# tg623623nana/Vehicle_Motion_Planning_with_Obstacles_Avoidance_using_MPC

Hardware: AMD Instinct MI355X
Metric: OBCA MPC steps/sec (batch) at N=5, 3 obs (higher is better)
Workload: dtype f64

## Files before the change

### vehicle_motion_planning_with_obstacles_avoidance_using_mpc_amd/csrc/obca_device.h

```cpp
#ifndef OBCA_DEVICE_H
#define OBCA_DEVICE_H

#include <math.h>
#include <stdint.h>
#include "../../include/obca_mpc.h"

#define OBCA_ACC_MAX0 0.6
#define OBCA_ACC_MAX1 0.5235987755982988
#define OBCA_T_MIN 1e-4

#define OBCA_MU_INIT 0.1
#define OBCA_KAPPA_MU 0.2
#define OBCA_THETA_MU 1.5
#define OBCA_KAPPA_EPS 10.0
#define OBCA_TAU_MIN 0.99
#define OBCA_BOUND_PUSH 1e-2
#define OBCA_BOUND_FRAC 1e-2
#define OBCA_KAPPA_D 1e-5
#define OBCA_KAPPA_SIGMA 1e10
#define OBCA_S_MAX 100.0
#define OBCA_GAMMA_THETA 1e-5
#define OBCA_GAMMA_PHI 1e-8
#define OBCA_DELTA 1.0
#define OBCA_S_THETA 1.1
// ... 72 lines not shown
    t += 4 * obca_even(N1) + 2 * obca_even(2 * np);
    t += 3 * obca_even(2 * np);
    t += obca_even(N1 * M * 2) + obca_even(N1 * M) + obca_even(3 * N1);
    t += obca_even(36 * N1) + obca_even(8 * N1);
    {
        const long long nx = obca_even(n_max), nr = obca_even(R_max), ny = (long long)MW * 4 * np;
        t += obca_even(ny > nx + nr ? ny : nx + nr);
    }
    t += obca_even(36 * N1 > 12 * np ? 36 * N1 : 12 * np) + obca_even(6 * N1) + obca_even(12 * N1) + obca_even(2 * N1) + obca_even(9 * (N1 + 1));
    t += obca_even(32) + obca_even(8);
    const int inst_off = (int)t;
    t += OBCA_INST_DOUBLES;
    return ObcaShapeSizes{n_max, R_max, inst_off, t};
}
#define OBCA_NO_MU_SLOT (1 << 20)
constexpr int obca_r_mu(int N, int nO, int M, int variant) {
    return 3 + 3 * N + (variant == 4 ? 3 : 0) + 2 * (N + 1) + 2 * N + 2 * N + (variant == 4 ? 2 : 0) + (variant == 6 ? 2 : 0) +
           2 * (N + 1) * nO + (N + 1) * M;
}
constexpr int obca_mu_slot(int N, int nO, int M, int nt) {
    int r = obca_r_mu(N, nO, M, 4);
    if (obca_r_mu(N, nO, M, 6) > r) r = obca_r_mu(N, nO, M, 6);
    if (obca_r_mu(N, nO, M, 8) > r) r = obca_r_mu(N, nO, M, 8);
    return (r + nt - 1) / nt;
}
static_assert(obca_mu_slot(5, 3, 6, 64) == 2 && obca_mu_slot(6, 3, 6, 64) == 3 && obca_mu_slot(5, 2, 2, 64) == 2 &&
              obca_mu_slot(5, 5, 14, 64) == 4 && obca_mu_slot(5, 6, 18, 64) == 4, "mu slots of the one-wavefront shapes");
static_assert(obca_mu_slot(20, 3, 6, 256) == 2 && obca_mu_slot(20, 5, 14, 256) == 3, "mu slots of the four-wavefront shapes");
#define OBCA_LDS_CU_BYTES (160 * 1024)
#define OBCA_LDS_STATIC_BYTES 64
constexpr long long obca_soc_doubles(int N, int nO, int M) {
    return obca_even((long long)obca_shape_sizes(N, nO, M).n_max + 2 * (long long)obca_shape_sizes(N, nO, M).R_max + 2 * (long long)(N + 1) * nO);
}
// ... 116 lines not shown
```

### vehicle_motion_planning_with_obstacles_avoidance_using_mpc_amd/csrc/obca_kernel.hip

```cpp

#include <hip/hip_runtime.h>
#include <stdint.h>
#include <math.h>
#include "obca_device.h"

#define SYNC() __syncthreads()

#ifndef OBCA_NT
#define OBCA_NT 64
#endif

#ifdef OBCA_PROFILE
#define PROF_DECL long long prof_last = wall_clock64();
#define PROF(i) { const long long t_ = wall_clock64(); prof_t[i] += t_ - prof_last; prof_last = t_; }
#define RPROF(i) { const long long t_ = wall_clock64(); prof_t[i] += t_ - rlast; rlast = t_; }
__device__ long long* prof_dummy;
#else
#define PROF_DECL
#define PROF(i)
#define RPROF(i)
#endif

namespace {

// ... 121 lines not shown
        const int k = pr / L.nO, i = pr - k * L.nO;
        const int o0 = S.offm[i], o1 = S.offm[i + 1];
        const double* lam = xv + L.il(k);
        const double* A = S.Aobs + (size_t)k * L.M * 2;
        double c0 = 0.0, c1 = 0.0;
        for (int j = o0; j < o1; ++j) {
            c0 += A[2 * j] * lam[j];
            c1 += A[2 * j + 1] * lam[j];
        }
        cc[2 * pr] = c0;
        cc[2 * pr + 1] = c1;
    }
    SYNC();
}

__device__ __forceinline__ double row_value(const Lay& L, const Sh& S, const Inst& in, const double* xv, const double* ct,
                            const double* st, const double* cc, int r) {
    const double T = L.free_T ? xv[L.iT()] : 1.0;
    const double h = T * in.Ts, ih = rcp64(h);
    if (r < L.r_dyn) return xv[r] - in.x0[r];
    if (r < L.r_term) {
        const int q = r - L.r_dyn, k = q / 3, j = q - 3 * k;
        const double* pk = xv + L.ip(k);
        const double* pn = xv + L.ip(k + 1);
        const double* u = xv + L.iu(k);
        const double f = (j == 0) ? u[0] * ct[k] : (j == 1) ? u[0] * st[k] : u[1];
        return pn[j] - pk[j] - h * f;
    }
    if (r < L.r_xb) {
        const int j = r - L.r_term;
        return xv[L.ip(L.N) + j] - S.xref[j * (L.N + 1) + L.N];
    }
    if (r < L.r_ub) {
        const int q = r - L.r_xb;
        return xv[L.ip(q >> 1) + (q & 1)];
    }
    if (r < L.r_acc) {
        const int q = r - L.r_ub;
        return xv[L.iu(q >> 1) + (q & 1)];
    }
    if (r < L.r_T) {
        const int q = r - L.r_acc, k = q >> 1, c = q & 1;
        const double prev = (k == 0) ? in.u0[c] : xv[L.iu(k - 1) + c];
        return (prev - xv[L.iu(k) + c]) * ih;
    }
    if (r < L.r_tx) return T;
    if (r < L.r_norm) return xv[L.ip(L.N) + (r - L.r_tx)];
    if (r < L.r_dist) {
        const int pr = r - L.r_norm;
        return cc[2 * pr] * cc[2 * pr] + cc[2 * pr + 1] * cc[2 * pr + 1];
    }
    if (r < L.r_lam) {
        const int pr = r - L.r_dist, k = pr / L.nO, i = pr - k * L.nO;
        const double* pk = xv + L.ip(k);
        const double tx = pk[0] + ct[k] * in.off, ty = pk[1] + st[k] * in.off;
        const double* mu = xv + L.imu(k) + 4 * i;
        const double* lam = xv + L.il(k);
        const double* b = S.bobs + (size_t)k * L.M;
        double v = -(in.gego[0] * mu[0] + in.gego[1] * mu[1] + in.gego[2] * mu[2] + in.gego[3] * mu[3]) +
                   tx * cc[2 * pr] + ty * cc[2 * pr + 1];
        for (int j = S.offm[i]; j < S.offm[i + 1]; ++j) v -= b[j] * lam[j];
        return v;
    }
    if (r < L.r_mu) {
        const int q = r - L.r_lam, k = q / L.M, j = q - k * L.M;
        return xv[L.il(k) + j];
    }
    {
        const int q = r - L.r_mu, w4 = 4 * L.nO, k = q / w4, j = q - k * w4;
        return xv[L.imu(k) + j];
    }
}

__device__ __forceinline__ void row_bounds(const Lay& L, const Inst& in, int r, double& lo, double& up) {
    const double INF = INFINITY;
    if (r < L.r_xb) { lo = 0.0; up = 0.0; return; }
    if (r < L.r_ub) { const int j = (r - L.r_xb) & 1; lo = in.xL[j]; up = in.xU[j]; return; }
    if (r < L.r_acc) { const int j = (r - L.r_ub) & 1; lo = in.uL[j]; up = in.uU[j]; return; }
    if (r < L.r_T) { const int c = (r - L.r_acc) & 1; const double a = c ? OBCA_ACC_MAX1 : OBCA_ACC_MAX0; lo = -a; up = a; return; }
    if (r < L.r_tx) { if (r == L.r_T) { lo = 0.0; up = INF; } else { lo = OBCA_T_MIN; up = in.Tmax; } return; }
    if (r < L.r_norm) { if (r == L.r_tx) { lo = in.term[0]; up = INF; } else { lo = in.term[1]; up = in.term[2]; } return; }
    if (r < L.r_dist) { lo = -INF; up = 1.0; return; }
    if (r < L.r_lam) { lo = in.dmin; up = INF; return; }
    lo = 0.0; up = INF;
}

__device__ __forceinline__ void rot_value(const Lay& L, const double* xv, const double* ct, const double* st,
                                          const double* cc, int pr, double& e1, double& e2) {
    const int k = pr / L.nO, i = pr - k * L.nO;
    const double* mu = xv + L.imu(k) + 4 * i;
    const double c0 = cc[2 * pr], c1 = cc[2 * pr + 1];
    e1 = mu[0] - mu[2] + ct[k] * c0 + st[k] * c1;
    e2 = mu[1] - mu[3] - st[k] * c0 + ct[k] * c1;
}

template <bool GRAD>
__device__ __forceinline__ double eval_objective(const Lay& L, const Sh& S, const Inst& in, const double* xv, double sf, int lane) {
    const double T = L.free_T ? xv[L.iT()] : 1.0;
// ... 132 lines not shown
            const double* yd = ym + L.r_dyn + 3 * k;
            double u0 = u[0], u1 = u[1], cs = S.ct[k], sn = S.st[k], yd0 = yd[0], yd1 = yd[1], yd2 = yd[2];
            double um0 = xv[L.iu(km)], um1 = xv[L.iu(km) + 1], ya0 = ym[L.r_acc + 2 * k], ya1 = ym[L.r_acc + 2 * k + 1];
            asm volatile("" : "+v"(u0), "+v"(u1), "+v"(cs), "+v"(sn), "+v"(yd0), "+v"(yd1), "+v"(yd2), "+v"(um0), "+v"(um1),
                              "+v"(ya0), "+v"(ya1), "+v"(gT), "+v"(yT0), "+v"(yT1));
            part -= in.Ts * (u0 * cs * yd0 + u0 * sn * yd1 + u1 * yd2);
            part -= ya0 * ((k == 0 ? in.u0[0] : um0) - u0) * iTh;
            part -= ya1 * ((k == 0 ? in.u0[1] : um1) - u1) * iTh;
        }
        part = red_sum(part);
        if (lane == 0) out[L.iT()] = gT + part + (L.N + 1) * (yT0 + yT1);
    }
    SYNC();
}

__device__ __forceinline__ double row_jdx(const Lay& L, const Sh& S, const Inst& in, int r) {
    const double* xv = S.x;
    const double* d = S.dx;
    const double T = L.free_T ? xv[L.iT()] : 1.0;
    const double dT = L.free_T ? d[L.iT()] : 0.0;
    const double h = T * in.Ts, ih = rcp64(h), iTh = ih * rcp64(T);
    if (r < L.r_xb) return d[L.ip(L.N) + (r - L.r_term)];
    if (r < L.r_ub) { const int q = r - L.r_xb; return d[L.ip(q >> 1) + (q & 1)]; }
    if (r < L.r_acc) { const int q = r - L.r_ub; return d[L.iu(q >> 1) + (q & 1)]; }
    if (r < L.r_T) {
        const int q = r - L.r_acc, k = q >> 1, c = q & 1;
        const double prev = (k == 0) ? in.u0[c] : xv[L.iu(k - 1) + c];
        const double dprev = (k == 0) ? 0.0 : d[L.iu(k - 1) + c];
        const double qq = prev - xv[L.iu(k) + c];
        return (dprev - d[L.iu(k) + c]) * ih - qq * iTh * dT;
    }
    if (r < L.r_tx) return dT;
    if (r < L.r_norm) return d[L.ip(L.N) + (r - L.r_tx)];
    if (r < L.r_lam) {
        const bool isn = r < L.r_dist;
        const int pr = isn ? r - L.r_norm : r - L.r_dist;
        const int k = pr / L.nO, i = pr - k * L.nO;
        const double c0 = S.cc[2 * pr], c1 = S.cc[2 * pr + 1];
        const double* A = S.Aobs + (size_t)k * L.M * 2;
        const double* dl = d + L.il(k);
        double s0 = 0.0, s1 = 0.0, sb = 0.0;
        for (int j = S.offm[i]; j < S.offm[i + 1]; ++j) {
            s0 += A[2 * j] * dl[j];
            s1 += A[2 * j + 1] * dl[j];
            sb += S.bobs[(size_t)k * L.M + j] * dl[j];
        }
        if (isn) return 2.0 * (c0 * s0 + c1 * s1);
        const double cs = S.ct[k], sn = S.st[k];
        const double* pk = xv + L.ip(k);
        const double* dp = d + L.ip(k);
        const double* dm = d + L.imu(k) + 4 * i;
        const double tx = pk[0] + cs * in.off, ty = pk[1] + sn * in.off;
        return -(in.gego[0] * dm[0] + in.gego[1] * dm[1] + in.gego[2] * dm[2] + in.gego[3] * dm[3]) + tx * s0 +
               ty * s1 - sb + c0 * dp[0] + c1 * dp[1] + in.off * (-sn * c0 + cs * c1) * dp[2];
    }
    if (r < L.r_mu) { const int q = r - L.r_lam, k = q / L.M; return d[L.il(k) + (q - k * L.M)]; }
    { const int q = r - L.r_mu, w4 = 4 * L.nO, k = q / w4; return d[L.imu(k) + (q - k * w4)]; }
}

#define OBCA_ROW_FIELDS(X) X(s) X(p) X(n) X(zL) X(zU) X(zp) X(zn) X(g) X(dy) X(iDs) X(iDp) X(iDn) X(rs) X(rp) X(rn)
template <int RPL>
struct Rows {
#define X(f) double f##_[RPL];
    OBCA_ROW_FIELDS(X)
#undef X
    __device__ __forceinline__ static constexpr int slots() { return RPL; }
#define X(f) __device__ __forceinline__ double& f(int j) { return f##_[j]; } \
             __device__ __forceinline__ double f(int j) const { return f##_[j]; }
    OBCA_ROW_FIELDS(X)
#undef X
};
// ... 1108 lines not shown
struct ObcaHead {
    int32_t B, N, nO, M, n_max, R_max, inst_off, two_sided, soc_lds;
    const int32_t* variant;
    const double *x0, *u0, *xref, *A, *b, *Ts, *term;
    double *xopt, *uopt, *ts_opt;
    int32_t *status, *iters;
    double *info, *prof, *warm_z;
    const int32_t* warm_use;
    double warm_mu;
    double *cert_z, *cert_y, *soc_ws, *gm_ws;
    long long gm_stride;
};

typedef const __attribute__((address_space(4))) ObcaLaunch ObcaLaunchConst;

struct ShapeAny { static constexpr bool fixed = false; static constexpr int N = 0, nO = 0, M = 0, n_max = 0, R_max = 0, inst_off = 0, soc_lds = 0, mu_slot = OBCA_NO_MU_SLOT; };
template <int N_, int NO_, int M_, bool FT = false>
struct ShapeIs {
    static constexpr bool fixed = true;
    static constexpr int N = N_, nO = NO_, M = M_;
    static constexpr int mu_slot = OBCA_NT == 64 ? obca_mu_slot(N_, NO_, M_, OBCA_NT) : OBCA_NO_MU_SLOT;
    static constexpr int n_max = obca_shape_sizes(N_, NO_, M_).n_max, R_max = obca_shape_sizes(N_, NO_, M_).R_max - (FT ? 3 : 0),
                         inst_off = obca_shape_sizes(N_, NO_, M_).inst_off;
#if OBCA_NT == 64
    static constexpr int RPL = R_max <= 256 ? 4 : R_max <= 320 ? 5 : 6;
    static_assert(R_max <= 384, "shape beyond the one-wavefront kernels");
    static constexpr int soc_lds = obca_soc_lds_wave(N_, NO_, M_);
#else
    static constexpr int RPL = R_max <= 768 ? 3 : -5;
    static_assert(R_max <= 1280, "shape beyond the four-wavefront LDS kernels");
    static constexpr int soc_lds = obca_soc_lds_mw(N_, NO_, M_);
#endif
};

template <int RPL, bool FROM_MEMORY = false, class DESC = const ObcaLaunch, class SHAPE = ShapeAny>
__device__ __forceinline__ void obca_ipm_body(DESC& Ain, const int inst, const bool first) {
    extern __shared__ __attribute__((aligned(16))) double smem[];
    const int lane = threadIdx.x;
    ObcaHead A;
    {
        constexpr bool U = FROM_MEMORY;
        A.B = uni<U>(Ain.B); A.N = uni<U>(Ain.N); A.nO = uni<U>(Ain.nO); A.M = uni<U>(Ain.M); A.n_max = uni<U>(Ain.n_max);
        A.R_max = uni<U>(Ain.R_max); A.inst_off = uni<U>(Ain.inst_off); A.two_sided = uni<U>(Ain.two_sided); A.soc_lds = uni<U>(Ain.soc_lds);
        A.variant = uni<U>(Ain.variant); A.x0 = uni<U>(Ain.x0); A.u0 = uni<U>(Ain.u0); A.xref = uni<U>(Ain.xref); A.A = uni<U>(Ain.A);
        A.b = uni<U>(Ain.b); A.Ts = uni<U>(Ain.Ts); A.term = uni<U>(Ain.term); A.xopt = uni<U>(Ain.xopt); A.uopt = uni<U>(Ain.uopt);
        A.ts_opt = uni<U>(Ain.ts_opt); A.status = uni<U>(Ain.status); A.iters = uni<U>(Ain.iters); A.info = uni<U>(Ain.info);
        A.prof = uni<U>(Ain.prof); A.warm_z = uni<U>(Ain.warm_z); A.warm_use = uni<U>(Ain.warm_use); A.warm_mu = uni<U>(Ain.warm_mu);
        A.cert_z = uni<U>(Ain.cert_z); A.cert_y = uni<U>(Ain.cert_y); A.soc_ws = uni<U>(Ain.soc_ws);
        A.gm_ws = Ain.gm_ws; A.gm_stride = Ain.gm_stride;
        if constexpr (SHAPE::fixed) {
            A.N = SHAPE::N; A.nO = SHAPE::nO; A.M = SHAPE::M; A.n_max = SHAPE::n_max; A.R_max = SHAPE::R_max; A.inst_off = SHAPE::inst_off;
            A.soc_lds = SHAPE::soc_lds;
        }
    }
    if (inst >= A.B) return;
#ifdef OBCA_PROFILE
    const long long prof_body_t0 = wall_clock64();
#endif
    if (A.variant[inst] == 0) {
        if (lane == 0) { A.status[inst] = OBCA_STATUS_SKIPPED; A.iters[inst] = 0; }
        return;
    }
    {
        const int v = A.variant[inst];
        if ((v != 4 && v != 6 && v != 8) || (v == 6 && A.term == nullptr)) {
            if (lane == 0 && first) { A.status[inst] = OBCA_STATUS_BAD_VARIANT; A.iters[inst] = 0; }
            return;
        }
    }
    __shared__ int ladder_state[4];
    __shared__ double ladder_f;
    const int order = OBCA_EFFECTIVE_ORDER(Ain.prm.opt.order, A.variant[inst], A.warm_z != nullptr && (A.warm_use == nullptr || A.warm_use[inst] != 0), Ain.prm.opt.nstarts == 1);
    int start_s = 0, escalated = 0, held_bits = 0;
    if (!first) {
        const int st0 = __builtin_amdgcn_readfirstlane(A.status[inst]);
        if (st0 == OBCA_STATUS_OK || st0 == OBCA_STATUS_ACCEPTABLE || st0 < OBCA_STATUS_NUMERIC) return;
        const int l0 = __builtin_amdgcn_readfirstlane(ladder_state[0]);
        escalated = l0 & 15; held_bits = l0 & 0xf20;
        start_s = __builtin_amdgcn_readfirstlane(ladder_state[3]);
        if (A.variant[inst] == 4 && (l0 & 16) && escalated < OBCA_N_ESCALATIONS) ++escalated;
        else { escalated = 0; if (++start_s >= Ain.prm.opt.nstarts + ((Ain.prm.opt.dodge && A.variant[inst] != 4) ? OBCA_DODGE_PASSES(A.variant[inst]) : 0)) return; }
    }
    const double rho_mult = escalated ? OBCA_RHO_ESCALATION(escalated) : 1.0;
    const int kind = start_s < Ain.prm.opt.nstarts ? OBCA_START_KIND(order, start_s) : (((start_s - Ain.prm.opt.nstarts) & 1) == 0 ? OBCA_KIND_DODGE_R : OBCA_KIND_DODGE_L);
    const bool dodge2 = start_s >= Ain.prm.opt.nstarts + 2;
    const bool from_window = kind == OBCA_KIND_WINDOW;

    Lay L;
    L.N = A.N; L.nO = A.nO; L.M = A.M;
    L.variant = A.variant[inst];
    L.free_T = (L.variant == 4) ? 1 : 0;
    L.NS = 5 + L.M + 4 * L.nO;
    L.n = (L.N + 1) * (3 + L.M + 4 * L.nO) + 2 * L.N + L.free_T;
    L.npair = (L.N + 1) * L.nO;
    L.r_init = 0; L.r_dyn = 3; L.r_term = 3 + 3 * L.N;
    L.r_xb = L.r_term + (L.variant == 4 ? 3 : 0);
    L.r_ub = L.r_xb + 2 * (L.N + 1);
    L.r_acc = L.r_ub + 2 * L.N;
    L.r_T = L.r_acc + 2 * L.N;
    L.r_tx = L.r_T + (L.free_T ? 2 : 0);
    L.r_norm = L.r_tx + (L.variant == 6 ? 2 : 0);
    L.r_dist = L.r_norm + L.npair;
    L.r_lam = L.r_dist + L.npair;
    L.r_mu = L.r_lam + (L.N + 1) * L.M;
    L.R = L.r_mu + (L.N + 1) * 4 * L.nO;

    constexpr bool GM = (RPL == 0);
    constexpr int MUS = SHAPE::mu_slot;
    Sh S;
    Rows<RPL> W;
    {
        double* p = smem;
        double* q = nullptr;
        if constexpr (GM) q = A.gm_ws + (size_t)blockIdx.x * (size_t)A.gm_stride;
        auto take = [&](int cnt) { double* r = p; p += (cnt + 1) & ~1; return r; };
        auto takeG = [&](int cnt) { if constexpr (!GM) { double* r = p; p += (cnt + 1) & ~1; return r; } else { double* r = q; q += (cnt + 1) & ~1; return r; } };
        const int nmax = A.n_max, Rmax = A.R_max, np = L.npair, N1 = L.N + 1;
        S.x = takeG(nmax); S.dx = takeG(nmax > 120 ? nmax : 120); S.gf = take(5 * N1 + 1); S.bx = takeG(nmax);
        S.y = takeG(Rmax); S.Einv = takeG(Rmax); S.gh = takeG(Rmax); S.Lb = takeG(Rmax); S.Ub = takeG(Rmax); S.dy = take(3 * N1 + 3);
        S.ct = take(N1); S.st = take(N1); S.cc = takeG(2 * np); S.ctt = take(N1); S.stt = take(N1); S.cct = takeG(2 * np);
// ... 125 lines not shown
    eval_geom(L, S, S.x, S.ct, S.st, S.cc, lane);
    double f0 = eval_objective<true>(L, S, in, S.x, 1.0, lane);
    {
        double gm = 0.0;
        for (int t = lane; t <= L.igT(); t += NT) gm = dmaxabs(gm, S.gf[t]);
        gm = fmax(red_max(gm), O.rho);
        sf = (gm > OBCA_MAX_GRADIENT) ? OBCA_MAX_GRADIENT / gm : 1.0;
        rho = O.rho * sf;
    }
    SYNC();
    f0 = eval_objective<true>(L, S, in, S.x, sf, lane);
    PUT(IV_F, f0);
    double mu = (from_window || (kind >= OBCA_KIND_DODGE_R && !dodge2)) ? OBCA_RESTART_MU : (warm ? A.warm_mu : (dodge2 ? OBCA_DODGE_LEVEL2_MU : OBCA_MU_INIT));
    {
        int bb = 0;
        for (int r = lane; r < L.R; r += NT) {
            double lo, up;
            row_bounds(L, in, r, lo, up);
            S.Lb[r] = lo; S.Ub[r] = up;
            S.tmp[r] = row_value(L, S, in, S.x, S.ct, S.st, S.cc, r);
        }
#pragma unroll
        for (int j = 0; j < W.slots(); ++j) {
            const int r = lane + NT * j;
            W.s(j) = 0.0; W.p(j) = 1.0; W.n(j) = 1.0;
            W.zL(j) = 0.0; W.zU(j) = 0.0; W.zp(j) = 1.0; W.zn(j) = 1.0; W.g(j) = 0.0; W.dy(j) = 0.0;
            W.iDs(j) = 0.0; W.iDp(j) = 1.0; W.iDn(j) = 1.0; W.rs(j) = 0.0; W.rp(j) = 0.0; W.rn(j) = 0.0;
            if (r < L.R) {
                const bool muk = mu_only<MUS>(j);
                const double lo = muk ? 0.0 : S.Lb[r], up = muk ? INFINITY : S.Ub[r];
// ... 199 lines not shown
            if (!bad || soc_pass) break;
            if (first_try) {
                delta_w = (dw_last == 0.0) ? OBCA_DELTA_W_0 : fmax(OBCA_DELTA_W_MIN, OBCA_KAPPA_W_MINUS * dw_last);
                first_try = false;
            } else {
                delta_w *= (dw_last == 0.0) ? OBCA_KAPPA_W_PLUS_BAR : OBCA_KAPPA_W_PLUS;
            }
            if (delta_w > OBCA_DELTA_W_MAX) { fail = 1; break; }
        }
        if (fail) { status = OBCA_STATUS_NUMERIC; break; }
        if (!soc_pass && delta_w > 0.0) PUT(IV_DWLAST, delta_w);
        double a_max = 1.0, a_z = 1.0, dphi = 0.0, phi = 0.0;
        const double phik = GET(IV_PHIK);
        const bool phi_known = !soc_pass && isfinite(phik);
        const double tau = GET(IV_TAU);
        for (int r = lane; r < L.R; r += NT)
            S.tmp[r] = row_soft(L, r) ? S.dy[r] : (row_jdx(L, S, in, r) + S.gh[r]) * S.Einv[r];
#if OBCA_NT == 64
        PROF(19)
#endif
#pragma unroll
        for (int j = 0; j < W.slots(); ++j) {
            const int r = lane + NT * j;
            if (r < L.R) {
                const bool muk = mu_only<MUS>(j);
                const bool eq = muk ? false : row_iseq(L, r);
                const double lo_ = muk ? 0.0 : S.Lb[r], up_ = muk ? INFINITY : S.Ub[r];
                const bool hasL = !eq && lo_ > -INFINITY, hasU = !eq && up_ < INFINITY;
                const double dy = S.tmp[r];
                W.dy(j) = dy;
// ... 58 lines not shown
        } else {
            a_try = a_max;
            a_z = S.lsv[LS_AZ]; dphi = S.lsv[LS_DPHI]; phi = S.lsv[LS_PHI]; alpha_min = S.lsv[LS_AMIN];
            pw_th = S.lsv[LS_PWTH]; pw_dphi = S.lsv[LS_PWDPHI]; alpha = S.lsv[LS_ALPHA]; th_old = S.lsv[LS_THOLD];
        }
        soc_pass = false;
        PROF(6)
        double f_t = 0.0, phi_acc = NAN;
        bool accepted = false, aug = false;
        for (;;) {
            for (int t = lane; t < L.n; t += NT) S.xt[t] = S.x[t] + a_try * S.dx[t];
            SYNC();
            eval_geom(L, S, S.xt, S.ctt, S.stt, S.cct, lane);
            f_t = eval_objective<true>(L, S, in, S.xt, sf, lane);
            double th_t = 0.0, phi_t = 0.0;
            for (int r = lane; r < L.R; r += NT) S.tmp[r] = row_value(L, S, in, S.xt, S.ctt, S.stt, S.cct, r);
#pragma unroll
            for (int j = 0; j < W.slots(); ++j) {
                const int r = lane + NT * j;
                if (r < L.R) {
                    const bool muk = mu_only<MUS>(j);
                    const bool eq = muk ? false : row_iseq(L, r);
                    const double dy = W.dy(j), w = muk ? 1.0 : row_w(L, r);
                    const double lo_ = muk ? 0.0 : S.Lb[r], up_ = muk ? INFINITY : S.Ub[r];
                    const double st = eq ? 0.0 : W.s(j) + a_try * (dy - W.rs(j)) * W.iDs(j);
                    const double pt = W.p(j) + a_try * (dy - W.rp(j)) * W.iDp(j);
                    const double nt = W.n(j) + a_try * (-dy - W.rn(j)) * W.iDn(j);
                    const double gt = S.tmp[r];
                    th_t += w * fabs(gt - st - pt + nt);
                    phi_t += w * row_barrier(lo_, up_, eq, st, pt, nt, mu, rho);
// ... 260 lines not shown
        const int NSs = 5 + a->M + 4 * a->nO, nn = N1 * (3 + a->M + 4 * a->nO) + 2 * a->N;
        for (int t = lane; t < nn; t += nt) { const int k = t / NSs, q = t - k * NSs; zc[t] = q < 3 ? x0s[q] : 0.0; }
    }
    if (a->cert_y != nullptr) {
        double* yc = a->cert_y + (size_t)inst * (a->R_max + 2 * N1 * a->nO);
        const int Rv = 3 + 3 * a->N + 2 * N1 + 4 * a->N + 2 + N1 * (2 * a->nO + a->M + 4 * a->nO);
        for (int t = lane; t < Rv + 2 * N1 * a->nO; t += nt) yc[t] = 0.0;
    }
    if (lane == 0) {
        a->ts_opt[inst] = ts; a->status[inst] = OBCA_STATUS_INFEASIBLE; a->iters[inst] = 0;
        if (a->info) { double* io = a->info + (size_t)inst * 4; io[0] = 0.0; io[1] = sh; io[2] = 0.0; io[3] = 0.0; }
    }
    return 1;
}

template <int RPL, bool LOOP, class DESC, class SHAPE = ShapeAny>
__device__ __forceinline__ void solve_passes(DESC& A, DESC& A2, DESC& A3) {
    const int inst = blockIdx.x;
    __shared__ int drv_scr;
    {
        extern __shared__ __attribute__((aligned(16))) double smem[];
        const int scr = terminal_screen_dev((const ObcaLaunch*)__builtin_amdgcn_kernarg_segment_ptr(), inst, threadIdx.x, blockDim.x,
                                            &reinterpret_cast<Inst*>(smem + A.inst_off)->Tmax);
        if (scr == 1) return;
        if (threadIdx.x == 0) drv_scr = scr;
    }
    if constexpr (LOOP) {
        if (inst >= A.B) return;
#pragma clang loop unroll(disable)
        for (int pass = 0; pass < OBCA_MAX_PASSES; ++pass) {
            obca_ipm_body<RPL, false, DESC, SHAPE>(A, inst, pass == 0);
            __syncthreads();
            const int st = A.status[inst];
            if (st == OBCA_STATUS_OK || st == OBCA_STATUS_ACCEPTABLE || st < OBCA_STATUS_NUMERIC) return;
            if (drv_scr == 2 && pass + 1 == A.prm.opt.nstarts) return;
        }
    } else {
        static_assert(OBCA_MAX_PASSES == 9, "one inlined copy of the body per pass");
        obca_ipm_body<RPL, false, DESC, SHAPE>(A, inst, true);
        if (inst >= A.B) return;
        __syncthreads();
        {
            const int st = A2.status[inst];
            if (st == OBCA_STATUS_OK || st == OBCA_STATUS_ACCEPTABLE || st < OBCA_STATUS_NUMERIC) return;
        }
        if (drv_scr == 2 && A2.prm.opt.nstarts == 1) return;
        obca_ipm_body<RPL, false, DESC, SHAPE>(A2, inst, false);
        __syncthreads();
        obca_ipm_body<RPL, false, DESC, SHAPE>(A3, inst, false);
        __syncthreads();
// ... 33 lines not shown
#ifndef OBCA_LOOP_GM
#define OBCA_LOOP_GM true
#endif
#if OBCA_NT == 64 && defined(OBCA_TU_SHAPE)
#ifndef OBCA_SHAPE_KERNEL_ATTR
#define OBCA_SHAPE_KERNEL_ATTR
#endif
#define OBCA_DEFINE_SHAPE_KERNEL(N_, O_, M_)                                                                                   \
    extern "C" __global__ void __launch_bounds__(64) OBCA_SHAPE_KERNEL_ATTR obca_ipm_kernel_s##N_##_##O_##_##M_(ObcaLaunch A, ObcaLaunch A2, ObcaLaunch A3) { \
        using SH = ShapeIs<N_, O_, M_>;                                                                                        \
        solve_with_escalation<SH::RPL, true, true, SH>(A, A2, A3);                                                            \
    }
OBCA_TU_SHAPE(OBCA_DEFINE_SHAPE_KERNEL)
#elif OBCA_NT == 64
extern "C" int obca_internal_mu_slot(int N, int nO, int M, int nt) { return obca_mu_slot(N, nO, M, nt); }
extern "C" __global__ void __launch_bounds__(64) obca_ipm_kernel_r4(ObcaLaunch A, ObcaLaunch A2, ObcaLaunch A3) { solve_with_escalation<4, OBCA_LOOP_R4>(A, A2, A3); }
extern "C" __global__ void __launch_bounds__(64) obca_ipm_kernel_r5(ObcaLaunch A, ObcaLaunch A2, ObcaLaunch A3) { solve_with_escalation<5, OBCA_LOOP_R56>(A, A2, A3); }
extern "C" __global__ void __launch_bounds__(64) obca_ipm_kernel_r6(ObcaLaunch A, ObcaLaunch A2, ObcaLaunch A3) { solve_with_escalation<6, OBCA_LOOP_R56>(A, A2, A3); }
extern "C" __global__ void __launch_bounds__(64) obca_ipm_kernel_gm1(ObcaLaunch A, ObcaLaunch A2, ObcaLaunch A3) { solve_with_escalation<0, OBCA_LOOP_GM>(A, A2, A3); }

#include "obca_rollout_core.h"
#include "obca_audit_core.h"

__device__ __noinline__ void ro_prepare(const rollout::Dev* D, int b) { rollout::prepare(*D, b); }
__device__ __noinline__ void ro_finish(const rollout::Dev* D, int b) { rollout::finish(*D, b); }
__device__ __noinline__ void ro_stop(const rollout::Dev* D, int b) { rollout::stop_check_wave(*D, b); }
__device__ __noinline__ int ro_screen(const ObcaLaunch* L, int b, double* tmax) { return terminal_screen_dev(L, b, 0, 1, tmax); }
__device__ __noinline__ int ro_retry(const rollout::Dev* D, int g, int b) { rollout::make_retry(*D, g, b); return D->var8[g][b]; }
__device__ __noinline__ long long ro_flag_sel(const rollout::Dev* D, int b) { return ((long long)D->sel[b] << 32) | (unsigned)D->flags[b]; }

// ... 173 lines not shown
```

Baseline: 1.206 million.

## Specialize IPM body per variant with compile-time row-kind dispatch

Adds per-variant template instantiations of the fixed-shape IPM body, so the row layout becomes compile-time constant. Row evaluation loops are split into a mixed prefix and a pure-mu tail, each with a compile-time mask of the row kinds it can hold. This lets the compiler drop impossible branches in row_value, row_bounds and row_jdx. It is meant to remove per-row branch chains and runtime layout arithmetic, at the cost of three inlined body copies, which adds code size and may raise register pressure.

```diff
diff --git a/vehicle_motion_planning_with_obstacles_avoidance_using_mpc_amd/csrc/obca_device.h b/vehicle_motion_planning_with_obstacles_avoidance_using_mpc_amd/csrc/obca_device.h
--- a/vehicle_motion_planning_with_obstacles_avoidance_using_mpc_amd/csrc/obca_device.h
+++ b/vehicle_motion_planning_with_obstacles_avoidance_using_mpc_amd/csrc/obca_device.h
@@ -110,9 +110,44 @@
     return ObcaShapeSizes{n_max, R_max, inst_off, t};
 }
 #define OBCA_NO_MU_SLOT (1 << 20)
-constexpr int obca_r_mu(int N, int nO, int M, int variant) {
-    return 3 + 3 * N + (variant == 4 ? 3 : 0) + 2 * (N + 1) + 2 * N + 2 * N + (variant == 4 ? 2 : 0) + (variant == 6 ? 2 : 0) +
-           2 * (N + 1) * nO + (N + 1) * M;
+struct ObcaRowLayout { int r_init, r_dyn, r_term, r_xb, r_ub, r_acc, r_T, r_tx, r_norm, r_dist, r_lam, r_mu, R, n, free_T; };
+constexpr ObcaRowLayout obca_row_layout(int N, int nO, int M, int variant) {
+    ObcaRowLayout l{};
+    l.free_T = variant == 4 ? 1 : 0;
+    l.n = (N + 1) * (3 + M + 4 * nO) + 2 * N + l.free_T;
+    l.r_init = 0; l.r_dyn = 3; l.r_term = 3 + 3 * N;
+    l.r_xb = l.r_term + (variant == 4 ? 3 : 0);
+    l.r_ub = l.r_xb + 2 * (N + 1);
+    l.r_acc = l.r_ub + 2 * N;
+    l.r_T = l.r_acc + 2 * N;
+    l.r_tx = l.r_T + (variant == 4 ? 2 : 0);
+    l.r_norm = l.r_tx + (variant == 6 ? 2 : 0);
+    l.r_dist = l.r_norm + (N + 1) * nO;
+    l.r_lam = l.r_dist + (N + 1) * nO;
+    l.r_mu = l.r_lam + (N + 1) * M;
+    l.R = l.r_mu + (N + 1) * 4 * nO;
+    return l;
+}
+constexpr int obca_r_mu(int N, int nO, int M, int variant) { return obca_row_layout(N, nO, M, variant).r_mu; }
+enum { OBCA_KIND_BIT_INIT = 1, OBCA_KIND_BIT_DYN = 2, OBCA_KIND_BIT_TERM = 4, OBCA_KIND_BIT_XB = 8, OBCA_KIND_BIT_UB = 16, OBCA_KIND_BIT_ACC = 32,
+       OBCA_KIND_BIT_T = 64, OBCA_KIND_BIT_TX = 128, OBCA_KIND_BIT_NORM = 256, OBCA_KIND_BIT_DIST = 512, OBCA_KIND_BIT_LAM = 1024,
+       OBCA_KIND_BIT_MU = 2048, OBCA_KIND_BITS_ALL = 4095 };
+constexpr int obca_slot_kinds(int N, int nO, int M, int variant, int nt, int j) {
+    const ObcaRowLayout l = obca_row_layout(N, nO, M, variant);
+    const int first[13] = {l.r_init, l.r_dyn, l.r_term, l.r_xb, l.r_ub, l.r_acc, l.r_T, l.r_tx, l.r_norm, l.r_dist, l.r_lam, l.r_mu, l.R};
+    const int lo = nt * j, hi = nt * j + nt < l.R ? nt * j + nt : l.R;
+    int kinds = 0;
+    for (int k = 0; k < 12; ++k) {
+        const int a = first[k] > lo ? first[k] : lo, b = first[k + 1] < hi ? first[k + 1] : hi;
+        if (a < b) kinds |= 1 << k;
+    }
+    return kinds;
+}
+constexpr int obca_own_mu_slot(int N, int nO, int M, int variant, int nt) { return (obca_r_mu(N, nO, M, variant) + nt - 1) / nt; }
+constexpr int obca_mixed_kinds(int N, int nO, int M, int variant, int nt) {
+    int kinds = 0;
+    for (int j = 0; j < obca_own_mu_slot(N, nO, M, variant, nt); ++j) kinds |= obca_slot_kinds(N, nO, M, variant, nt, j);
+    return kinds;
 }
 constexpr int obca_mu_slot(int N, int nO, int M, int nt) {
     int r = obca_r_mu(N, nO, M, 4);
diff --git a/vehicle_motion_planning_with_obstacles_avoidance_using_mpc_amd/csrc/obca_kernel.hip b/vehicle_motion_planning_with_obstacles_avoidance_using_mpc_amd/csrc/obca_kernel.hip
--- a/vehicle_motion_planning_with_obstacles_avoidance_using_mpc_amd/csrc/obca_kernel.hip
+++ b/vehicle_motion_planning_with_obstacles_avoidance_using_mpc_amd/csrc/obca_kernel.hip
@@ -2,6 +2,7 @@
 #include <hip/hip_runtime.h>
 #include <stdint.h>
 #include <math.h>
+#include <type_traits>
 #include "obca_device.h"
 
 #define SYNC() __syncthreads()
@@ -159,12 +160,18 @@
     SYNC();
 }
 
+#define OBCA_ROW_IS(K, bound) ((KM & (K)) != 0 && ((KM & ~(2 * (K) - 1)) == 0 || r < (bound)))
+template <int KM = OBCA_KIND_BITS_ALL>
 __device__ __forceinline__ double row_value(const Lay& L, const Sh& S, const Inst& in, const double* xv, const double* ct,
                             const double* st, const double* cc, int r) {
+    if constexpr (KM == OBCA_KIND_BIT_MU) {
+        const int q = r - L.r_mu, w4 = 4 * L.nO, k = q / w4, j = q - k * w4;
+        return xv[L.imu(k) + j];
+    }
     const double T = L.free_T ? xv[L.iT()] : 1.0;
     const double h = T * in.Ts, ih = rcp64(h);
-    if (r < L.r_dyn) return xv[r] - in.x0[r];
-    if (r < L.r_term) {
+    if (OBCA_ROW_IS(OBCA_KIND_BIT_INIT, L.r_dyn)) return xv[r] - in.x0[r];
+    if (OBCA_ROW_IS(OBCA_KIND_BIT_DYN, L.r_term)) {
         const int q = r - L.r_dyn, k = q / 3, j = q - 3 * k;
         const double* pk = xv + L.ip(k);
         const double* pn = xv + L.ip(k + 1);
@@ -172,30 +179,30 @@
         const double f = (j == 0) ? u[0] * ct[k] : (j == 1) ? u[0] * st[k] : u[1];
         return pn[j] - pk[j] - h * f;
     }
-    if (r < L.r_xb) {
+    if (OBCA_ROW_IS(OBCA_KIND_BIT_TERM, L.r_xb)) {
         const int j = r - L.r_term;
         return xv[L.ip(L.N) + j] - S.xref[j * (L.N + 1) + L.N];
     }
-    if (r < L.r_ub) {
+    if (OBCA_ROW_IS(OBCA_KIND_BIT_XB, L.r_ub)) {
         const int q = r - L.r_xb;
         return xv[L.ip(q >> 1) + (q & 1)];
     }
-    if (r < L.r_acc) {
+    if (OBCA_ROW_IS(OBCA_KIND_BIT_UB, L.r_acc)) {
         const int q = r - L.r_ub;
         return xv[L.iu(q >> 1) + (q & 1)];
     }
-    if (r < L.r_T) {
+    if (OBCA_ROW_IS(OBCA_KIND_BIT_ACC, L.r_T)) {
         const int q = r - L.r_acc, k = q >> 1, c = q & 1;
         const double prev = (k == 0) ? in.u0[c] : xv[L.iu(k - 1) + c];
         return (prev - xv[L.iu(k) + c]) * ih;
     }
-    if (r < L.r_tx) return T;
-    if (r < L.r_norm) return xv[L.ip(L.N) + (r - L.r_tx)];
-    if (r < L.r_dist) {
+    if (OBCA_ROW_IS(OBCA_KIND_BIT_T, L.r_tx)) return T;
+    if (OBCA_ROW_IS(OBCA_KIND_BIT_TX, L.r_norm)) return xv[L.ip(L.N) + (r - L.r_tx)];
+    if (OBCA_ROW_IS(OBCA_KIND_BIT_NORM, L.r_dist)) {
         const int pr = r - L.r_norm;
         return cc[2 * pr] * cc[2 * pr] + cc[2 * pr + 1] * cc[2 * pr + 1];
     }
-    if (r < L.r_lam) {
+    if (OBCA_ROW_IS(OBCA_KIND_BIT_DIST, L.r_lam)) {
         const int pr = r - L.r_dist, k = pr / L.nO, i = pr - k * L.nO;
         const double* pk = xv + L.ip(k);
         const double tx = pk[0] + ct[k] * in.off, ty = pk[1] + st[k] * in.off;
@@ -207,7 +214,7 @@
         for (int j = S.offm[i]; j < S.offm[i + 1]; ++j) v -= b[j] * lam[j];
         return v;
     }
-    if (r < L.r_mu) {
+    if (OBCA_ROW_IS(OBCA_KIND_BIT_LAM, L.r_mu)) {
         const int q = r - L.r_lam, k = q / L.M, j = q - k * L.M;
         return xv[L.il(k) + j];
     }
@@ -217,16 +224,18 @@
     }
 }
 
+template <int KM = OBCA_KIND_BITS_ALL>
 __device__ __forceinline__ void row_bounds(const Lay& L, const Inst& in, int r, double& lo, double& up) {
     const double INF = INFINITY;
-    if (r < L.r_xb) { lo = 0.0; up = 0.0; return; }
-    if (r < L.r_ub) { const int j = (r - L.r_xb) & 1; lo = in.xL[j]; up = in.xU[j]; return; }
-    if (r < L.r_acc) { const int j = (r - L.r_ub) & 1; lo = in.uL[j]; up = in.uU[j]; return; }
-    if (r < L.r_T) { const int c = (r - L.r_acc) & 1; const double a = c ? OBCA_ACC_MAX1 : OBCA_ACC_MAX0; lo = -a; up = a; return; }
-    if (r < L.r_tx) { if (r == L.r_T) { lo = 0.0; up = INF; } else { lo = OBCA_T_MIN; up = in.Tmax; } return; }
-    if (r < L.r_norm) { if (r == L.r_tx) { lo = in.term[0]; up = INF; } else { lo = in.term[1]; up = in.term[2]; } return; }
-    if (r < L.r_dist) { lo = -INF; up = 1.0; return; }
-    if (r < L.r_lam) { lo = in.dmin; up = INF; return; }
+    constexpr int EQ = OBCA_KIND_BIT_INIT | OBCA_KIND_BIT_DYN | OBCA_KIND_BIT_TERM;
+    if ((KM & EQ) != 0 && ((KM & ~EQ) == 0 || r < L.r_xb)) { lo = 0.0; up = 0.0; return; }
+    if (OBCA_ROW_IS(OBCA_KIND_BIT_XB, L.r_ub)) { const int j = (r - L.r_xb) & 1; lo = in.xL[j]; up = in.xU[j]; return; }
+    if (OBCA_ROW_IS(OBCA_KIND_BIT_UB, L.r_acc)) { const int j = (r - L.r_ub) & 1; lo = in.uL[j]; up = in.uU[j]; return; }
+    if (OBCA_ROW_IS(OBCA_KIND_BIT_ACC, L.r_T)) { const int c = (r - L.r_acc) & 1; const double a = c ? OBCA_ACC_MAX1 : OBCA_ACC_MAX0; lo = -a; up = a; return; }
+    if (OBCA_ROW_IS(OBCA_KIND_BIT_T, L.r_tx)) { if (r == L.r_T) { lo = 0.0; up = INF; } else { lo = OBCA_T_MIN; up = in.Tmax; } return; }
+    if (OBCA_ROW_IS(OBCA_KIND_BIT_TX, L.r_norm)) { if (r == L.r_tx) { lo = in.term[0]; up = INF; } else { lo = in.term[1]; up = in.term[2]; } return; }
+    if (OBCA_ROW_IS(OBCA_KIND_BIT_NORM, L.r_dist)) { lo = -INF; up = 1.0; return; }
+    if (OBCA_ROW_IS(OBCA_KIND_BIT_DIST, L.r_lam)) { lo = in.dmin; up = INF; return; }
     lo = 0.0; up = INF;
 }
 
@@ -389,26 +398,28 @@
     SYNC();
 }
 
+template <int KM = OBCA_KIND_BITS_ALL>
 __device__ __forceinline__ double row_jdx(const Lay& L, const Sh& S, const Inst& in, int r) {
     const double* xv = S.x;
     const double* d = S.dx;
+    if constexpr (KM == OBCA_KIND_BIT_MU) { const int q = r - L.r_mu, w4 = 4 * L.nO, k = q / w4; return d[L.imu(k) + (q - k * w4)]; }
     const double T = L.free_T ? xv[L.iT()] : 1.0;
     const double dT = L.free_T ? d[L.iT()] : 0.0;
     const double h = T * in.Ts, ih = rcp64(h), iTh = ih * rcp64(T);
-    if (r < L.r_xb) return d[L.ip(L.N) + (r - L.r_term)];
-    if (r < L.r_ub) { const int q = r - L.r_xb; return d[L.ip(q >> 1) + (q & 1)]; }
-    if (r < L.r_acc) { const int q = r - L.r_ub; return d[L.iu(q >> 1) + (q & 1)]; }
-    if (r < L.r_T) {
+    if (OBCA_ROW_IS(OBCA_KIND_BIT_TERM, L.r_xb)) return d[L.ip(L.N) + (r - L.r_term)];
+    if (OBCA_ROW_IS(OBCA_KIND_BIT_XB, L.r_ub)) { const int q = r - L.r_xb; return d[L.ip(q >> 1) + (q & 1)]; }
+    if (OBCA_ROW_IS(OBCA_KIND_BIT_UB, L.r_acc)) { const int q = r - L.r_ub; return d[L.iu(q >> 1) + (q & 1)]; }
+    if (OBCA_ROW_IS(OBCA_KIND_BIT_ACC, L.r_T)) {
         const int q = r - L.r_acc, k = q >> 1, c = q & 1;
         const double prev = (k == 0) ? in.u0[c] : xv[L.iu(k - 1) + c];
         const double dprev = (k == 0) ? 0.0 : d[L.iu(k - 1) + c];
         const double qq = prev - xv[L.iu(k) + c];
         return (dprev - d[L.iu(k) + c]) * ih - qq * iTh * dT;
     }
-    if (r < L.r_tx) return dT;
-    if (r < L.r_norm) return d[L.ip(L.N) + (r - L.r_tx)];
-    if (r < L.r_lam) {
-        const bool isn = r < L.r_dist;
+    if (OBCA_ROW_IS(OBCA_KIND_BIT_T, L.r_tx)) return dT;
+    if (OBCA_ROW_IS(OBCA_KIND_BIT_TX, L.r_norm)) return d[L.ip(L.N) + (r - L.r_tx)];
+    if ((KM & (OBCA_KIND_BIT_NORM | OBCA_KIND_BIT_DIST)) != 0 && ((KM & (OBCA_KIND_BIT_LAM | OBCA_KIND_BIT_MU)) == 0 || r < L.r_lam)) {
+        const bool isn = (KM & OBCA_KIND_BIT_NORM) != 0 && ((KM & OBCA_KIND_BIT_DIST) == 0 || r < L.r_dist);
         const int pr = isn ? r - L.r_norm : r - L.r_dist;
         const int k = pr / L.nO, i = pr - k * L.nO;
         const double c0 = S.cc[2 * pr], c1 = S.cc[2 * pr + 1];
@@ -429,7 +440,7 @@
         return -(in.gego[0] * dm[0] + in.gego[1] * dm[1] + in.gego[2] * dm[2] + in.gego[3] * dm[3]) + tx * s0 +
                ty * s1 - sb + c0 * dp[0] + c1 * dp[1] + in.off * (-sn * c0 + cs * c1) * dp[2];
     }
-    if (r < L.r_mu) { const int q = r - L.r_lam, k = q / L.M; return d[L.il(k) + (q - k * L.M)]; }
+    if (OBCA_ROW_IS(OBCA_KIND_BIT_LAM, L.r_mu)) { const int q = r - L.r_lam, k = q / L.M; return d[L.il(k) + (q - k * L.M)]; }
     { const int q = r - L.r_mu, w4 = 4 * L.nO, k = q / w4; return d[L.imu(k) + (q - k * w4)]; }
 }
 
@@ -1568,11 +1579,17 @@
 
 typedef const __attribute__((address_space(4))) ObcaLaunch ObcaLaunchConst;
 
-struct ShapeAny { static constexpr bool fixed = false; static constexpr int N = 0, nO = 0, M = 0, n_max = 0, R_max = 0, inst_off = 0, soc_lds = 0, mu_slot = OBCA_NO_MU_SLOT; };
-template <int N_, int NO_, int M_, bool FT = false>
+struct ShapeAny {
+    static constexpr bool fixed = false, per_variant = false;
+    static constexpr int N = 0, nO = 0, M = 0, n_max = 0, R_max = 0, inst_off = 0, soc_lds = 0, mu_slot = OBCA_NO_MU_SLOT, variant = 0;
+};
+template <int N_, int NO_, int M_, bool FT = false, int V_ = 0>
 struct ShapeIs {
+    static_assert(V_ == 0 || V_ == 4 || V_ == 6 || V_ == 8, "variant: 4, 6, 8 or 0 (run time)");
     static constexpr bool fixed = true;
-    static constexpr int N = N_, nO = NO_, M = M_;
+    static constexpr int N = N_, nO = NO_, M = M_, variant = V_;
+    static constexpr bool per_variant = OBCA_NT == 64 && !FT && V_ == 0;
+    template <int V> using with_variant = ShapeIs<N_, NO_, M_, FT, V>;
     static constexpr int mu_slot = OBCA_NT == 64 ? obca_mu_slot(N_, NO_, M_, OBCA_NT) : OBCA_NO_MU_SLOT;
     static constexpr int n_max = obca_shape_sizes(N_, NO_, M_).n_max, R_max = obca_shape_sizes(N_, NO_, M_).R_max - (FT ? 3 : 0),
                          inst_off = obca_shape_sizes(N_, NO_, M_).inst_off;
@@ -1586,6 +1603,17 @@
     static constexpr int soc_lds = obca_soc_lds_mw(N_, NO_, M_);
 #endif
 };
+
+template <class SHAPE, class F>
+__device__ __forceinline__ void mixed_then_mu(int lane, F f) {
+    constexpr ObcaRowLayout K = obca_row_layout(SHAPE::N, SHAPE::nO, SHAPE::M, SHAPE::variant);
+    constexpr int MUSV = obca_own_mu_slot(SHAPE::N, SHAPE::nO, SHAPE::M, SHAPE::variant, NT), MIXED = NT * MUSV < K.R ? NT * MUSV : K.R;
+    constexpr int MIX = obca_mixed_kinds(SHAPE::N, SHAPE::nO, SHAPE::M, SHAPE::variant, NT);
+#pragma unroll 1
+    for (int r = lane; r < MIXED; r += NT) f(std::integral_constant<int, MIX>{}, r);
+#pragma unroll 1
+    for (int r = lane + NT * MUSV; r < K.R; r += NT) f(std::integral_constant<int, OBCA_KIND_BIT_MU>{}, r);
+}
 
 template <int RPL, bool FROM_MEMORY = false, class DESC = const ObcaLaunch, class SHAPE = ShapeAny>
 __device__ __forceinline__ void obca_ipm_body(DESC& Ain, const int inst, const bool first) {
@@ -1611,20 +1639,23 @@
 #ifdef OBCA_PROFILE
     const long long prof_body_t0 = wall_clock64();
 #endif
-    if (A.variant[inst] == 0) {
-        if (lane == 0) { A.status[inst] = OBCA_STATUS_SKIPPED; A.iters[inst] = 0; }
-        return;
-    }
-    {
-        const int v = A.variant[inst];
-        if ((v != 4 && v != 6 && v != 8) || (v == 6 && A.term == nullptr)) {
-            if (lane == 0 && first) { A.status[inst] = OBCA_STATUS_BAD_VARIANT; A.iters[inst] = 0; }
+    auto variant_of = [&]() __attribute__((always_inline)) -> int { if constexpr (SHAPE::variant != 0) return SHAPE::variant; else return A.variant[inst]; };
+    if constexpr (SHAPE::variant == 0) {
+        if (A.variant[inst] == 0) {
+            if (lane == 0) { A.status[inst] = OBCA_STATUS_SKIPPED; A.iters[inst] = 0; }
             return;
+        }
+        {
+            const int v = A.variant[inst];
+            if ((v != 4 && v != 6 && v != 8) || (v == 6 && A.term == nullptr)) {
+                if (lane == 0 && first) { A.status[inst] = OBCA_STATUS_BAD_VARIANT; A.iters[inst] = 0; }
+                return;
+            }
         }
     }
     __shared__ int ladder_state[4];
     __shared__ double ladder_f;
-    const int order = OBCA_EFFECTIVE_ORDER(Ain.prm.opt.order, A.variant[inst], A.warm_z != nullptr && (A.warm_use == nullptr || A.warm_use[inst] != 0), Ain.prm.opt.nstarts == 1);
+    const int order = OBCA_EFFECTIVE_ORDER(Ain.prm.opt.order, variant_of(), A.warm_z != nullptr && (A.warm_use == nullptr || A.warm_use[inst] != 0), Ain.prm.opt.nstarts == 1);
     int start_s = 0, escalated = 0, held_bits = 0;
     if (!first) {
         const int st0 = __builtin_amdgcn_readfirstlane(A.status[inst]);
@@ -1632,8 +1663,8 @@
         const int l0 = __builtin_amdgcn_readfirstlane(ladder_state[0]);
         escalated = l0 & 15; held_bits = l0 & 0xf20;
         start_s = __builtin_amdgcn_readfirstlane(ladder_state[3]);
-        if (A.variant[inst] == 4 && (l0 & 16) && escalated < OBCA_N_ESCALATIONS) ++escalated;
-        else { escalated = 0; if (++start_s >= Ain.prm.opt.nstarts + ((Ain.prm.opt.dodge && A.variant[inst] != 4) ? OBCA_DODGE_PASSES(A.variant[inst]) : 0)) return; }
+        if (variant_of() == 4 && (l0 & 16) && escalated < OBCA_N_ESCALATIONS) ++escalated;
+        else { escalated = 0; if (++start_s >= Ain.prm.opt.nstarts + ((Ain.prm.opt.dodge && variant_of() != 4) ? OBCA_DODGE_PASSES(variant_of()) : 0)) return; }
     }
     const double rho_mult = escalated ? OBCA_RHO_ESCALATION(escalated) : 1.0;
     const int kind = start_s < Ain.prm.opt.nstarts ? OBCA_START_KIND(order, start_s) : (((start_s - Ain.prm.opt.nstarts) & 1) == 0 ? OBCA_KIND_DODGE_R : OBCA_KIND_DODGE_L);
@@ -1642,7 +1673,7 @@
 
     Lay L;
     L.N = A.N; L.nO = A.nO; L.M = A.M;
-    L.variant = A.variant[inst];
+    L.variant = variant_of();
     L.free_T = (L.variant == 4) ? 1 : 0;
     L.NS = 5 + L.M + 4 * L.nO;
     L.n = (L.N + 1) * (3 + L.M + 4 * L.nO) + 2 * L.N + L.free_T;
@@ -1658,6 +1689,12 @@
     L.r_lam = L.r_dist + L.npair;
     L.r_mu = L.r_lam + (L.N + 1) * L.M;
     L.R = L.r_mu + (L.N + 1) * 4 * L.nO;
+    if constexpr (SHAPE::variant != 0) {
+        constexpr ObcaRowLayout K = obca_row_layout(SHAPE::N, SHAPE::nO, SHAPE::M, SHAPE::variant);
+        L.free_T = K.free_T; L.n = K.n;
+        L.r_init = K.r_init; L.r_dyn = K.r_dyn; L.r_term = K.r_term; L.r_xb = K.r_xb; L.r_ub = K.r_ub; L.r_acc = K.r_acc; L.r_T = K.r_T;
+        L.r_tx = K.r_tx; L.r_norm = K.r_norm; L.r_dist = K.r_dist; L.r_lam = K.r_lam; L.r_mu = K.r_mu; L.R = K.R;
+    }
 
     constexpr bool GM = (RPL == 0);
     constexpr int MUS = SHAPE::mu_slot;
@@ -1813,6 +1850,15 @@
     double mu = (from_window || (kind >= OBCA_KIND_DODGE_R && !dodge2)) ? OBCA_RESTART_MU : (warm ? A.warm_mu : (dodge2 ? OBCA_DODGE_LEVEL2_MU : OBCA_MU_INIT));
     {
         int bb = 0;
+        if constexpr (SHAPE::variant != 0) {
+            mixed_then_mu<SHAPE>(lane, [&](auto km, int r) __attribute__((always_inline)) {
+                constexpr int KM = decltype(km)::value;
+                double lo, up;
+                row_bounds<KM>(L, in, r, lo, up);
+                S.Lb[r] = lo; S.Ub[r] = up;
+                S.tmp[r] = row_value<KM>(L, S, in, S.x, S.ct, S.st, S.cc, r);
+            });
+        } else
         for (int r = lane; r < L.R; r += NT) {
             double lo, up;
             row_bounds(L, in, r, lo, up);
@@ -2042,6 +2088,13 @@
         const double phik = GET(IV_PHIK);
         const bool phi_known = !soc_pass && isfinite(phik);
         const double tau = GET(IV_TAU);
+        if constexpr (SHAPE::variant != 0) {
+            mixed_then_mu<SHAPE>(lane, [&](auto km, int r) __attribute__((always_inline)) {
+                constexpr int KM = decltype(km)::value, SOFT = OBCA_KIND_BIT_INIT | OBCA_KIND_BIT_DYN;
+                const bool soft = (KM & SOFT) != 0 && ((KM & ~SOFT) == 0 || row_soft(L, r));
+                S.tmp[r] = soft ? S.dy[r] : (row_jdx<KM>(L, S, in, r) + S.gh[r]) * S.Einv[r];
+            });
+        } else
         for (int r = lane; r < L.R; r += NT)
             S.tmp[r] = row_soft(L, r) ? S.dy[r] : (row_jdx(L, S, in, r) + S.gh[r]) * S.Einv[r];
 #if OBCA_NT == 64
@@ -2130,6 +2183,11 @@
             eval_geom(L, S, S.xt, S.ctt, S.stt, S.cct, lane);
             f_t = eval_objective<true>(L, S, in, S.xt, sf, lane);
             double th_t = 0.0, phi_t = 0.0;
+            if constexpr (SHAPE::variant != 0) {
+                mixed_then_mu<SHAPE>(lane, [&](auto km, int r) __attribute__((always_inline)) {
+                    S.tmp[r] = row_value<decltype(km)::value>(L, S, in, S.xt, S.ctt, S.stt, S.cct, r);
+                });
+            } else
             for (int r = lane; r < L.R; r += NT) S.tmp[r] = row_value(L, S, in, S.xt, S.ctt, S.stt, S.cct, r);
 #pragma unroll
             for (int j = 0; j < W.slots(); ++j) {
@@ -2420,6 +2478,17 @@
     return 1;
 }
 
+template <int RPL, class DESC, class SHAPE>
+__device__ __forceinline__ void pass_loop(DESC& A, const int inst, const int* drv_scr) {
+#pragma clang loop unroll(disable)
+    for (int pass = 0; pass < OBCA_MAX_PASSES; ++pass) {
+        obca_ipm_body<RPL, false, DESC, SHAPE>(A, inst, pass == 0);
+        __syncthreads();
+        const int st = A.status[inst];
+        if (st == OBCA_STATUS_OK || st == OBCA_STATUS_ACCEPTABLE || st < OBCA_STATUS_NUMERIC) return;
+        if (*drv_scr == 2 && pass + 1 == A.prm.opt.nstarts) return;
+    }
+}
 template <int RPL, bool LOOP, class DESC, class SHAPE = ShapeAny>
 __device__ __forceinline__ void solve_passes(DESC& A, DESC& A2, DESC& A3) {
     const int inst = blockIdx.x;
@@ -2433,13 +2502,24 @@
     }
     if constexpr (LOOP) {
         if (inst >= A.B) return;
+        if constexpr (SHAPE::per_variant) {
+            const int v = A.variant[inst];
+            if (v == 0 || (v != 4 && v != 6 && v != 8) || (v == 6 && A.term == nullptr)) {
+                if (threadIdx.x == 0) { A.status[inst] = v == 0 ? OBCA_STATUS_SKIPPED : OBCA_STATUS_BAD_VARIANT; A.iters[inst] = 0; }
+                return;
+            }
+            if (v == 4) pass_loop<RPL, DESC, typename SHAPE::template with_variant<4>>(A, inst, &drv_scr);
+            else if (v == 6) pass_loop<RPL, DESC, typename SHAPE::template with_variant<6>>(A, inst, &drv_scr);
+            else pass_loop<RPL, DESC, typename SHAPE::template with_variant<8>>(A, inst, &drv_scr);
+        } else {
 #pragma clang loop unroll(disable)
-        for (int pass = 0; pass < OBCA_MAX_PASSES; ++pass) {
-            obca_ipm_body<RPL, false, DESC, SHAPE>(A, inst, pass == 0);
-            __syncthreads();
-            const int st = A.status[inst];
-            if (st == OBCA_STATUS_OK || st == OBCA_STATUS_ACCEPTABLE || st < OBCA_STATUS_NUMERIC) return;
-            if (drv_scr == 2 && pass + 1 == A.prm.opt.nstarts) return;
+            for (int pass = 0; pass < OBCA_MAX_PASSES; ++pass) {
+                obca_ipm_body<RPL, false, DESC, SHAPE>(A, inst, pass == 0);
+                __syncthreads();
+                const int st = A.status[inst];
+                if (st == OBCA_STATUS_OK || st == OBCA_STATUS_ACCEPTABLE || st < OBCA_STATUS_NUMERIC) return;
+                if (drv_scr == 2 && pass + 1 == A.prm.opt.nstarts) return;
+            }
         }
     } else {
         static_assert(OBCA_MAX_PASSES == 9, "one inlined copy of the body per pass");
@@ -2503,6 +2583,14 @@
 OBCA_TU_SHAPE(OBCA_DEFINE_SHAPE_KERNEL)
 #elif OBCA_NT == 64
 extern "C" int obca_internal_mu_slot(int N, int nO, int M, int nt) { return obca_mu_slot(N, nO, M, nt); }
+extern "C" void obca_internal_row_layout(int N, int nO, int M, int variant, int* out) {
+    const ObcaRowLayout l = obca_row_layout(N, nO, M, variant);
+    const int f[15] = {l.r_init, l.r_dyn, l.r_term, l.r_xb, l.r_ub, l.r_acc, l.r_T, l.r_tx, l.r_norm, l.r_dist, l.r_lam, l.r_mu, l.R, l.n, l.free_T};
+    for (int i = 0; i < 15; ++i) out[i] = f[i];
+}
+extern "C" int obca_internal_slot_kinds(int N, int nO, int M, int variant, int nt, int j) { return obca_slot_kinds(N, nO, M, variant, nt, j); }
+extern "C" int obca_internal_own_mu_slot(int N, int nO, int M, int variant, int nt) { return obca_own_mu_slot(N, nO, M, variant, nt); }
+extern "C" int obca_internal_mixed_kinds(int N, int nO, int M, int variant, int nt) { return obca_mixed_kinds(N, nO, M, variant, nt); }
 extern "C" __global__ void __launch_bounds__(64) obca_ipm_kernel_r4(ObcaLaunch A, ObcaLaunch A2, ObcaLaunch A3) { solve_with_escalation<4, OBCA_LOOP_R4>(A, A2, A3); }
 extern "C" __global__ void __launch_bounds__(64) obca_ipm_kernel_r5(ObcaLaunch A, ObcaLaunch A2, ObcaLaunch A3) { solve_with_escalation<5, OBCA_LOOP_R56>(A, A2, A3); }
 extern "C" __global__ void __launch_bounds__(64) obca_ipm_kernel_r6(ObcaLaunch A, ObcaLaunch A2, ObcaLaunch A3) { solve_with_escalation<6, OBCA_LOOP_R56>(A, A2, A3); }
```

Result: faster. 1.275 million, median of 6 (+5.7%).
